# jamornsriwasansak/evplp

Hardware: AMD Instinct MI355X
Metric: Mpaths/s (higher is better)
Workload: dtype f32

## Files before the change

### evplp_amd/csrc/device_common.hpp

```cpp
#pragma once
#include "evplp_types.h"
#include "ev_math.h"

namespace evplp {

#define EV_PI 3.14159265358979323846f
#define EV_INV_PI 0.318309886183790671537767526745028724068919291480912897495f
#define EV_DEV __device__ __forceinline__

struct V3 { float x, y, z; };
EV_DEV V3 v3(float x, float y, float z) { V3 r; r.x = x; r.y = y; r.z = z; return r; }
EV_DEV V3 v3(const float *p) { return v3(p[0], p[1], p[2]); }
EV_DEV V3 v3(float4 a) { return v3(a.x, a.y, a.z); }
EV_DEV V3 operator+(V3 a, V3 b) { return v3(a.x + b.x, a.y + b.y, a.z + b.z); }
EV_DEV V3 operator-(V3 a, V3 b) { return v3(a.x - b.x, a.y - b.y, a.z - b.z); }
EV_DEV V3 operator-(V3 a) { return v3(-a.x, -a.y, -a.z); }
EV_DEV V3 operator*(V3 a, V3 b) { return v3(a.x * b.x, a.y * b.y, a.z * b.z); }
EV_DEV V3 operator*(V3 a, float s) { return v3(a.x * s, a.y * s, a.z * s); }
EV_DEV V3 operator/(V3 a, float s) { return v3(a.x / s, a.y / s, a.z / s); }
EV_DEV float dot(V3 a, V3 b) { return a.x * b.x + a.y * b.y + a.z * b.z; }
EV_DEV V3 cross(V3 a, V3 b) { return v3(a.y * b.z - a.z * b.y, a.z * b.x - a.x * b.z, a.x * b.y - a.y * b.x); }
EV_DEV V3 normalize(V3 v) { float inv = 1.0f / sqrtf(dot(v, v)); return v * inv; }
EV_DEV V3 reflect(V3 i, V3 n) { float d = dot(n, i); return i - (n * 2.0f) * d; }
EV_DEV V3 faceforward(V3 n, V3 i, V3 nref) { return n * copysignf(1.0f, dot(i, nref)); }
// ... 386 lines not shown
        "v_pk_fma_f32 " T0 ", %[hx], %[pb], " T0 " op_sel:[0,1,0] op_sel_hi:[1,1,1]\n\t"                                                                                     \
        "v_pk_fma_f32 " T1 ", %[hy], %[pc], " T1 " op_sel:[0,0,0] op_sel_hi:[1,0,1]\n\t"                                                                                     \
        "v_pk_fma_f32 " T2 ", %[hz], %[pc], " T2 " op_sel:[0,1,0] op_sel_hi:[1,1,1]\n\t"                                                                                     \
        "v_max3_f32 " T3L ", " T3L ", " T4L ", " T5L " clamp\n\t"                                                                            \
        "v_min3_f32 " T0L ", " T0L ", " T1L ", " T2L " clamp\n\t"                                                                            \
        "v_max3_f32 " T3H ", " T3H ", " T4H ", " T5H " clamp\n\t"                                                                            \
        "v_min3_f32 " T0H ", " T0H ", " T1H ", " T2H " clamp\n\t"                                                                            \
        "v_cmp_lt_f32 vcc, " T3L ", " T0L "\n\t"                                                                                             \
        "v_cmp_lt_f32 %[m1], " T3H ", " T0H "\n\t"                                                                                           \
        "s_or_b64 %[t64], vcc, %[m1]\n\t"                                                                                                    \
        "s_cbranch_scc0 L_pop%=\n\t"                                                                                                         \
        "s_cmp_eq_u64 vcc, 0\n\t"                                                                                                            \
        "s_cbranch_scc1 L_c1%=\n\t"                                                                                                          \
        "s_cmp_eq_u64 %[m1], 0\n\t"                                                                                                          \
        "s_cbranch_scc1 L_c0%=\n\t"                                                                                                          \
        "s_bcnt1_i32_b64 %[p0], vcc\n\t"                                                                                                     \
        "s_bcnt1_i32_b64 %[p1], %[m1]\n\t"                                                                                                   \
        "s_cmp_ge_i32 %[p0], %[p1]\n\t"                                                                                                      \
        "s_cselect_b32 %[p0], %[c1], %[c0]\n\t"                                                                                              \
        "s_cselect_b32 %[cur], %[c0], %[c1]\n\t"                                                                                             \
        "s_mov_b32 m0, %[sp]\n\t"                                                                                                            \
        "s_add_i32 %[sp], %[sp], 1\n\t"                                                                                                      \
        "v_writelane_b32 %[vstack], %[p0], m0\n\t"                                                                                           \
        "s_branch L_end%=\n"                                                                                                                 \
        "L_c0%=:\n\t"                                                                                                                        \
        "s_mov_b32 %[cur], %[c0]\n\t"                                                                                                        \
        "s_branch L_end%=\n"                                                                                                                 \
        "L_c1%=:\n\t"                                                                                                                        \
        "s_mov_b32 %[cur], %[c1]\n\t"                                                                                                        \
        "s_branch L_end%=\n"                                                                                                                 \
        "L_pop%=:\n\t"                                                                                                                       \
        "s_brev_b32 %[cur], 1\n\t"                                                                                                           \
        "s_cmp_eq_u32 %[sp], 0\n\t"                                                                                                          \
        "s_cbranch_scc1 L_end%=\n\t"                                                                                                         \
        "s_sub_i32 %[sp], %[sp], 1\n\t"                                                                                                      \
        "s_nop 0\n\t"                                                                                                                        \
        "v_readlane_b32 %[cur], %[vstack], %[sp]\n"                                                                                          \
        "L_end%=:\n"                                                                                                                         \
        : [cur] "+s"(cur), [sp] "+s"(sp), [vstack] "+v"(vstack), [m1] "=&s"(m1_), [t64] "=&s"(t64_), [p0] "=&s"(p0_), [p1] "=&s"(p1_)          \
        : [cx] NC(cx_), [cy] NC(cy_), [cz] NC(cz_), [hx] NC(hx_), [hy] NC(hy_), [hz] NC(hz_), [c0] "s"(c0_), [c1] "s"(c1_),              \
          [pa] "v"(pa_), [pb] "v"(pb_), [pc] "v"(pc_),                                     \
          [pd] "v"(pd_), [pe] "v"(pe_), [lane] "v"(lane_id)                                                                 \
        : "vcc", "scc", "m0", T0L, T0H, T1L, T1H, T2L, T2H, T3L, T3H, T4L, T4H, T5L, T5H)

template <int VT = 0, bool CUT = false>
EV_DEV bool occluded_wave(const char *node_base, const char *leaf_base, V3 o, V3 d, float tmin, float tmax, bool alive_lane, WalkStats *ws = nullptr, const char *cut = nullptr, uint32_t cut_off = 0u,
                          const float4 *cut_lds = nullptr) {
    unsigned long long alive = ballot64(alive_lane), hitm = 0ull;
    if (alive == 0ull) return false;
    uint32_t cut_end = 0u;
    constexpr bool kCutLds = CUT && VT != 0 && EVPLP_WALK_ASM && !EVPLP_TRAVERSAL_STATS;
    if constexpr (kCutLds) {
        const int32_t nsyn = __builtin_amdgcn_readfirstlane(__float_as_int(cut_lds[3].z));
        if (nsyn == 0) return false;
        cut_off = 0u; cut_end = (uint32_t)nsyn;
    } else if constexpr (CUT) {
        int32_t nsyn;
        asm volatile("s_load_dword %0, %1, %2 offset:0x38\n\ts_waitcnt lgkmcnt(0)" : "=s"(nsyn) : "s"(cut), "s"(cut_off) : "memory");
        if (nsyn == 0) return false;
        cut_end = cut_off + ((uint32_t)nsyn << 6);
    }
    const V3 inv0 = v3(safe_rcp(d.x), safe_rcp(d.y), safe_rcp(d.z));
    const float ku = 1.0f / (tmax - tmin);
    const V3 inv = inv0 * ku;
    const v2f ivx = bc(inv.x), ivy = bc(inv.y), ivz = bc(inv.z);
    const v2f avx = bc(fabsf(inv.x)), avy = bc(fabsf(inv.y)), avz = bc(fabsf(inv.z));
    const float dead = __builtin_inff();
    v2f nox = bc(alive_lane ? (-(o.x * inv0.x) - tmin) * ku : dead), noy = bc(alive_lane ? (-(o.y * inv0.y) - tmin) * ku : dead),
        noz = bc(alive_lane ? (-(o.z * inv0.z) - tmin) * ku : dead);
    int sp = 0;
    int vstack = 0;
    int32_t cur = 0;
#if EVPLP_WALK_ASM && !EVPLP_TRAVERSAL_STATS
    if constexpr (VT != 0) {
        static_assert(VT == 52 || VT == 116, "reserved temporaries: v[52:63] or v[116:127]");
        const int lane_id = (int)(threadIdx.x & 63u);
        v2f pa_, pb_, pc_, pd_, pe_;
        pa_.x = ivx.x; pa_.y = ivy.x; pb_.x = ivz.x; pb_.y = avx.x; pc_.x = avy.x; pc_.y = avz.x;
        pd_.x = nox.x; pd_.y = noy.x; pe_.x = noz.x; pe_.y = noz.x;
#define EV_VISIT(N)                                                                                                                          \
        {                                                                                                                                    \
            const v2f cx_ = pk(N[0], N[1]), cy_ = pk(N[2], N[3]), cz_ = pk(N[4], N[5]), hx_ = pk(N[6], N[7]), hy_ = pk(N[8], N[9]), hz_ = pk(N[10], N[11]); \
            const int32_t c0_ = N[12], c1_ = N[13];                                                                                          \
            unsigned long long m1_, t64_; int32_t p0_, p1_;                                                                                  \
            if constexpr (VT == 52) EV_WALK_VISIT_ASM("v[52:53]", "v[54:55]", "v[56:57]", "v[58:59]", "v[60:61]", "v[62:63]", "v52", "v53", "v54", "v55", "v56", "v57", "v58", "v59", "v60", "v61", "v62", "v63"); \
            else EV_WALK_VISIT_ASM("v[116:117]", "v[118:119]", "v[120:121]", "v[122:123]", "v[124:125]", "v[126:127]", "v116", "v117", "v118", "v119", "v120", "v121", "v122", "v123", "v124", "v125", "v126", "v127"); \
        }
        for (;;) {
            if constexpr (CUT) {
                if (cut_off >= cut_end) break;
                v16i syn;
                {
                    const float4 *q = cut_lds + 4u * cut_off;
#pragma unroll
                    for (int w = 0; w < 4; w++) {
                        const float4 qq = q[w];
                        if (w < 3 || true) { syn[4 * w] = __builtin_amdgcn_readfirstlane(__float_as_int(qq.x)); syn[4 * w + 1] = __builtin_amdgcn_readfirstlane(__float_as_int(qq.y)); }
                        if (w < 3) { syn[4 * w + 2] = __builtin_amdgcn_readfirstlane(__float_as_int(qq.z)); syn[4 * w + 3] = __builtin_amdgcn_readfirstlane(__float_as_int(qq.w)); }
                    }
                    syn[14] = 0; syn[15] = 0;
                }
                cut_off++;
                EV_VISIT(syn)
            }
            for (;;) {
                while (cur >= 0) {
                    const v16i n = sload16(node_base, (uint32_t)cur << 6);
                    EV_VISIT(n)
                }
                if (cur == kNoChild) break;
                const uint32_t cnt = (((uint32_t)~cur) & 3u) + 1u, loff = (((uint32_t)~cur) >> 2) * 192u;
                bool any;
// ... 448 lines not shown
```

### evplp_amd/csrc/kernels.h

```cpp
#pragma once
#include "evplp_types.h"

namespace evplp {

struct PrimaryArgs {
    SceneDev sc; StripDev st; CamBasis cam;
    float jitter[2]; int32_t clear_light; int32_t pad;
    float4 *g_pos, *g_nrm, *g_dif, *g_phg, *g_light;
    float4 *tile_box;
    const char *cuts; int32_t cut_gw_log2, cut_gh_log2, cut_groups_x, pad2;
};
struct PrimaryCutArgs {
    const BvhNode *nodes; StripDev st; CamBasis cam;
    int32_t tiles_x, tiles_y, gw_log2, gh_log2, groups_x, groups_y;
    char *cuts;
};
void launch_primary_cuts(const PrimaryCutArgs &a, hipStream_t s);

struct LightTraceArgs {
    SceneDev sc;
    uint32_t rng_seed, path_begin, path_count, photons_per_path;
    evplp_record *records;
    int32_t *stack_overflow;
    uint32_t overflow_stride, pad;
};
#ifndef EVPLP_LT_STACK
#define EVPLP_LT_STACK 20
#endif
constexpr int kLtLdsStack = EVPLP_LT_STACK;
inline int lt_overflow_entries(const SceneDev &sc) {
    const int generic = 3 * ((sc.bvh_depth + 1) / 2) + 4;
    const int worst = sc.stack4_entries > 0 && sc.stack4_entries < generic ? sc.stack4_entries : generic;
    return worst > kLtLdsStack ? worst - kLtLdsStack : 0;
}

struct PassCounters {
    unsigned long long rays;
    unsigned long long nodes;
    unsigned long long pairs;
    unsigned long long aux;
    unsigned long long hist[64];
    unsigned long long shard_rays[64], shard_shaded[64];
    unsigned long long nonfinite;
};
#ifndef EVPLP_DEBUG_NAN
#define EVPLP_DEBUG_NAN 0
#endif
constexpr int kCounterShards = 64;

struct GatherArgs {
    SceneDev sc; StripDev st;
    const float4 *g_pos, *g_nrm, *g_dif, *g_phg;
    const evplp_record *vpls;
    const uint32_t *vpl_src_index;
    const uint32_t *nvpl;
    evplp_frame_params fp;
    float pdf_mc2; int32_t pad0;
    float4 *out;
    float4 *partial;
    size_t partial_stride;
    PassCounters *counters;
    int32_t splits_per_wave;
    int32_t block_h_log2;
    int32_t group_first, group_count;
    unsigned long long *vsl_masks; int32_t masks_per_split; int32_t pad1;
    const char *cuts; uint32_t cut_vpl_stride; int32_t cut_gw_log2, cut_gh_log2, cut_groups_x;
    int32_t band_first, band_rows, cut_group_row_first;
    int32_t item_deal;
    unsigned long long *block_cost;
};
struct AdaptArgs { const int4 *tiles; const float4 *snap; int32_t n1, pad; };
constexpr int kCutEntries = 8;
constexpr int kCutNodes = kCutEntries / 2;
constexpr int kCutSlotBytes = kCutNodes * 64;
struct CutArgs {
    const BvhNode *nodes;
    const float4 *tile_box;
    int32_t tiles_x, tiles_y;
    int32_t gw_log2, gh_log2;
    int32_t groups_x, groups_y;
    int32_t group_row_first, pad;
    const evplp_record *vpls; const uint32_t *nvpl; uint32_t vpl_stride;
    char *cuts;
    const int4 *adapt_tiles;
};
void launch_gather_cuts(const CutArgs &a, hipStream_t s);
void launch_tile_boxes(const StripDev &st, const float4 *g_pos, float4 *tile_box, int tiles_x, int tiles_y, hipStream_t s);
#ifndef EVPLP_VPL_SPLIT
#define EVPLP_VPL_SPLIT 128
#endif
constexpr int kVplSplit = EVPLP_VPL_SPLIT;
#ifndef EVPLP_GATHER_K
#define EVPLP_GATHER_K 2
#endif
constexpr int kDefaultSplitsPerWave = EVPLP_GATHER_K;

struct PathTraceArgs {
    SceneDev sc; StripDev st;
    const float4 *g_pos, *g_nrm, *g_dif, *g_phg;
    float camera_pos[3]; uint32_t rng_seed;
    uint32_t max_bounces, do_accumulate;
    float4 *out;
    PassCounters *counters;
};

constexpr int kPtBatchMaxSamples = 64;
constexpr size_t kPtBatchSlotBytes = 4 * 64 * sizeof(float4);
struct PtBatchSamples { float jitter[kPtBatchMaxSamples][2]; uint32_t seed[kPtBatchMaxSamples]; };
struct PtBatchChunk {
    const int32_t *list, *count;
    int32_t tiles;
    int32_t entry_first, entry_count, sample_first, sample_count, pad;
    float4 *staging;
    unsigned long long cut_mask;
};
void launch_pt_batch_list(const int4 *tiles, int32_t ntiles, int32_t *list, int32_t *count, hipStream_t s);
void launch_pt_batch_primary(const PrimaryArgs &a, const PtBatchSamples &sm, const PtBatchChunk &ch, hipStream_t s);
void launch_pt_batch_trace(const PathTraceArgs &a, const PtBatchSamples &sm, const PtBatchChunk &ch, hipStream_t s);
void launch_pt_batch_reduce(const StripDev &st, float4 *out, const PtBatchChunk &ch, hipStream_t s);
void launch_pt_batch_rescale(const StripDev &st, float4 *out, const AdaptArgs &ad, int32_t ntiles, hipStream_t s);

constexpr int kPtBudgetMaxTiles = 1 << 25;
struct PtBudgetChunk {
    const uint32_t *table; const int32_t *total;
    int32_t item_first, item_count;
    float4 *staging;
    unsigned long long cut_mask;
// ... 115 lines not shown
```

### evplp_amd/csrc/kernels_cut.hip

```cpp
#include "device_common.hpp"
#include "kernels.h"

namespace evplp {

struct CutFrustum {
    V3 p;
    float lo[3], hi[3];
    V3 pl[4]; float tol[4];
    bool planes;
};
EV_DEV bool cut_outside(const CutFrustum &F, const float c[3], const float h[3]) {
    bool out = false;
#pragma unroll
    for (int k = 0; k < 3; k++) out = out || (c[k] - h[k] > F.hi[k]) || (c[k] + h[k] < F.lo[k]);
    if (F.planes) {
        const V3 rel = v3(c[0] - F.p.x, c[1] - F.p.y, c[2] - F.p.z);
        const float mag = fabsf(rel.x) + fabsf(rel.y) + fabsf(rel.z) + h[0] + h[1] + h[2];
#pragma unroll
        for (int q = 0; q < 4; q++) {
            const V3 n = F.pl[q];
            const float far = __builtin_fmaf(fabsf(n.z), h[2], __builtin_fmaf(fabsf(n.y), h[1], __builtin_fmaf(fabsf(n.x), h[0], __builtin_fmaf(n.z, rel.z, __builtin_fmaf(n.y, rel.y, n.x * rel.x)))));
            out = out || (__builtin_fmaf(mag, F.tol[q], far) < 0.0f);
        }
    }
// ... 76 lines not shown
#pragma unroll
                for (int e = 0; e < 2; e++) {
                    if (2 * s2 + e < count) box_of(order[2 * s2 + e], c[e], h[e], r[e]);
                    else { r[e] = kNoChild; c[e][0] = c[e][1] = c[e][2] = 0.f; h[e][0] = h[e][1] = h[e][2] = -3.0e38f; }
                }
                out[4 * s2 + 0] = make_float4(c[0][0], c[1][0], c[0][1], c[1][1]);
                out[4 * s2 + 1] = make_float4(c[0][2], c[1][2], h[0][0], h[1][0]);
                out[4 * s2 + 2] = make_float4(h[0][1], h[1][1], h[0][2], h[1][2]);
                out[4 * s2 + 3] = make_float4(__int_as_float(r[0]), __int_as_float(r[1]), __int_as_float(nsyn), 0.f);
            }
        }
    }
}

template <bool ADAPT = false>
__global__ __launch_bounds__(64) void gather_cut_kernel(CutArgs a) {
    __shared__ int32_t s_ref[kCutRing][64];
    __shared__ uint32_t s_src[kCutRing][64];
    const int lane = threadIdx.x;
    const uint32_t nvpl = *a.nvpl;
    const uint32_t i = blockIdx.x % a.vpl_stride, gb = blockIdx.x / a.vpl_stride;
    if (i >= nvpl) return;
    const int gblocks_x = (a.groups_x + 7) >> 3;
    const int gx = (int)(gb % (uint32_t)gblocks_x) * 8 + (lane & 7), gyl = (int)(gb / (uint32_t)gblocks_x) * 8 + (lane >> 3);
    bool live = gx < a.groups_x && gyl < a.groups_y;
    if constexpr (ADAPT) {
        if (live) {
            const int gw = 1 << a.gw_log2, gh = 1 << a.gh_log2, gyi = a.group_row_first + gyl;
            bool retired = true;
            for (int ty = gyi * gh; ty < min((gyi + 1) * gh, a.tiles_y); ty++)
                for (int tx = gx * gw; tx < min((gx + 1) * gw, a.tiles_x); tx++) retired = retired && a.adapt_tiles[ty * a.tiles_x + tx].x != 0;
            live = !retired;
        }
    }
    if (__builtin_amdgcn_ballot_w64(live) == 0ull) return;
    const uint32_t g = (uint32_t)(min(gyl, a.groups_y - 1) * a.groups_x + min(gx, a.groups_x - 1));
    const int gy = a.group_row_first + min(gyl, a.groups_y - 1);
    const int gxc = min(gx, a.groups_x - 1);
    const float4 pv = reinterpret_cast<const float4 *>(a.vpls + i)[0];
    CutFrustum F; F.p = v3(pv.x, pv.y, pv.z);

    const int gw = 1 << a.gw_log2, gh = 1 << a.gh_log2;
    float ulo[3] = { 3.0e38f, 3.0e38f, 3.0e38f }, uhi[3] = { -3.0e38f, -3.0e38f, -3.0e38f };
    for (int ty = gy * gh; ty < min((gy + 1) * gh, a.tiles_y); ty++)
        for (int tx = gxc * gw; tx < min((gxc + 1) * gw, a.tiles_x); tx++) {
            const float4 lo = a.tile_box[2 * (ty * a.tiles_x + tx)], hi = a.tile_box[2 * (ty * a.tiles_x + tx) + 1];
            if (lo.x > hi.x) continue;
            ulo[0] = fminf(ulo[0], lo.x); ulo[1] = fminf(ulo[1], lo.y); ulo[2] = fminf(ulo[2], lo.z);
            uhi[0] = fmaxf(uhi[0], hi.x); uhi[1] = fmaxf(uhi[1], hi.y); uhi[2] = fmaxf(uhi[2], hi.z);
        }
    const bool any_tile = ulo[0] <= uhi[0];
    char *const slot = a.cuts + ((size_t)g * a.vpl_stride + i) * (size_t)kCutSlotBytes;
    if (live && !any_tile) reinterpret_cast<float4 *>(slot)[3] = make_float4(0.f, 0.f, 0.f, 0.f);
    const bool work = live && any_tile;
    if (!any_tile) { ulo[0] = ulo[1] = ulo[2] = 0.f; uhi[0] = uhi[1] = uhi[2] = 0.f; }
    {
        const float pp[3] = { F.p.x, F.p.y, F.p.z };
#pragma unroll
        for (int k = 0; k < 3; k++) {
            const float t0 = 0.0001f, t1 = 1.0f - 0.0001f;
            const float a0 = pp[k] * (1.0f - t0) + t0 * ulo[k], b0 = pp[k] * (1.0f - t0) + t0 * uhi[k];
            const float a1 = pp[k] * (1.0f - t1) + t1 * ulo[k], b1 = pp[k] * (1.0f - t1) + t1 * uhi[k];
            const float l = fminf(a0, a1), h = fmaxf(b0, b1);
            const float pad = 1.0e-5f * ((h - l) + fabsf(l) + fabsf(h)) + 1.0e-30f;
            F.lo[k] = l - pad; F.hi[k] = h + pad;
        }
    }
    {
        const V3 cen = v3(0.5f * (ulo[0] + uhi[0]), 0.5f * (ulo[1] + uhi[1]), 0.5f * (ulo[2] + uhi[2]));
        V3 m = cen - F.p;
        const float ml2 = dot(m, m);
        bool planes = ml2 > 1.0e-30f;
        m = m * __builtin_amdgcn_rsqf(fmaxf(ml2, 1.0e-30f));
        const V3 ax = fabsf(m.x) < 0.6f ? v3(1.f, 0.f, 0.f) : v3(0.f, 1.f, 0.f);
        V3 u = cross(m, ax); u = u * __builtin_amdgcn_rsqf(fmaxf(dot(u, u), 1.0e-30f));
        const V3 w = cross(m, u);
        float amin = 3.0e38f, amax = -3.0e38f, bmin = 3.0e38f, bmax = -3.0e38f;
#pragma unroll
        for (int q = 0; q < 8; q++) {
            const V3 d = v3(((q & 1) ? uhi[0] : ulo[0]) - F.p.x, ((q & 2) ? uhi[1] : ulo[1]) - F.p.y, ((q & 4) ? uhi[2] : ulo[2]) - F.p.z);
            const float dw = dot(m, d), dl2 = dot(d, d);
            if (!(dw > 0.0f) || dw * dw <= 0.0025f * dl2) planes = false;
            const float r = __builtin_amdgcn_rcpf(dw);
            const float ca = dot(u, d) * r, cb = dot(w, d) * r;
            amin = fminf(amin, ca); amax = fmaxf(amax, ca); bmin = fminf(bmin, cb); bmax = fmaxf(bmax, cb);
        }
        const float oa = 1.0e-4f * (1.0f + fmaxf(fabsf(amin), fabsf(amax))), ob = 1.0e-4f * (1.0f + fmaxf(fabsf(bmin), fabsf(bmax)));
        amin -= oa; amax += oa; bmin -= ob; bmax += ob;
        F.planes = planes;
        F.pl[0] = u - m * amin; F.pl[1] = m * amax - u; F.pl[2] = w - m * bmin; F.pl[3] = m * bmax - w;
#pragma unroll
        for (int q = 0; q < 4; q++) F.tol[q] = 4.0e-6f * (fabsf(F.pl[q].x) + fabsf(F.pl[q].y) + fabsf(F.pl[q].z));
    }

    cut_descend_and_store(a.nodes, F, slot, work, lane, s_ref, s_src);
}

__global__ __launch_bounds__(64) void primary_cut_kernel(PrimaryCutArgs a) {
    __shared__ int32_t s_ref[kCutRing][64];
    __shared__ uint32_t s_src[kCutRing][64];
    const int lane = threadIdx.x;
    const int gblocks_x = (a.groups_x + 7) >> 3;
    const int gx = (int)(blockIdx.x % (uint32_t)gblocks_x) * 8 + (lane & 7), gy = (int)(blockIdx.x / (uint32_t)gblocks_x) * 8 + (lane >> 3);
    const bool live = gx < a.groups_x && gy < a.groups_y;
    const int gxc = min(gx, a.groups_x - 1), gyc = min(gy, a.groups_y - 1);
    const int gw = 8 << a.gw_log2, gh = 8 << a.gh_log2;
    const int x0 = gxc * gw, x1 = min(x0 + gw, a.st.W) - 1;
// ... 30 lines not shown
```

### evplp_amd/csrc/kernels_gather.hip

```cpp
#include "device_common.hpp"
#include "kernels.h"
#include <algorithm>

namespace evplp {

constexpr int kRecF4 = sizeof(evplp_record) / 16;

struct Pixel {
    V3 p1, n1, rd, rs; float e; V3 wi10;
};

struct Vpl {
    V3 pos, n, flux, fdir, rd, rs; float psel, e;
};
EV_DEV Vpl load_vpl(const float4 *r) {
    Vpl v; float4 a = r[0], b = r[1], c = r[2], d = r[3], e = r[4], f = r[5];
    v.pos = v3(a); v.n = v3(b); v.psel = b.w; v.flux = v3(c); v.fdir = v3(d); v.rd = v3(e); v.rs = v3(f); v.e = f.w;
    return v;
}

EV_DEV float phong_eval_f_hw(V3 out, V3 in, V3 n, float e) {
    V3 r = reflect(-in, n);
    float d = fmaxf(dot(out, r), 0.0f);
    if (d <= 0.000001f) return 0.0f;
// ... 88 lines not shown
    return t;
}

template <bool RANGE = false>
EV_DEV uint32_t item_texel(const GatherArgs &a, int lane, int b) {
    const StripDev &st = a.st;
    const ItemIx ix = item_index<RANGE>(a, b);
    const int x = ix.tx * 8 + (lane & 7), ly = ix.ty * 8 + (lane >> 3);
    return (uint32_t)max(min(ly, st.local_rows - 1), 0) * (uint32_t)st.W + (uint32_t)min(x, st.W - 1);
}

EV_DEV uint32_t item_cut_group(const GatherArgs &a, const Item &t) {
    const int tx = __builtin_amdgcn_readfirstlane(t.x) >> 3, ty = __builtin_amdgcn_readfirstlane(t.ly) >> 3;
    return (uint32_t)(((ty >> a.cut_gh_log2) - a.cut_group_row_first) * a.cut_groups_x + (tx >> a.cut_gw_log2));
}
EV_DEV bool tile_retired(const GatherArgs &a, const AdaptArgs &ad, const Item &t) {
    const int tx = __builtin_amdgcn_readfirstlane(t.x) >> 3, ty = __builtin_amdgcn_readfirstlane(t.ly) >> 3;
    const uint32_t off = (uint32_t)(ty * ((a.st.W + 7) >> 3) + tx) * (uint32_t)sizeof(int4);
    int nt;
    asm volatile("s_load_dword %0, %1, %2\n\ts_waitcnt lgkmcnt(0)" : "=s"(nt) : "s"(ad.tiles), "s"(off) : "memory");
    return nt != 0;
}

#ifndef EVPLP_CUT_RING
#define EVPLP_CUT_RING 3
#endif
#ifndef EVPLP_PX_LDS
#define EVPLP_PX_LDS 1
#endif
constexpr int kGatherPxFloats = 64 * (EVPLP_PX_LDS ? 10 : 3);
#ifndef EVPLP_GATHER_WAVES
#define EVPLP_GATHER_WAVES 8
#endif

EV_DEV Vpl fetch_vpl(const evplp_record *r) {
    const v16i ra = *reinterpret_cast<const v16i *>(r);
    const v8i rb = *reinterpret_cast<const v8i *>(reinterpret_cast<const int *>(r) + 16);
    Vpl v;
    v.pos = v3(f_of(ra[0]), f_of(ra[1]), f_of(ra[2])); v.n = v3(f_of(ra[4]), f_of(ra[5]), f_of(ra[6])); v.psel = f_of(ra[7]);
    v.flux = v3(f_of(ra[8]), f_of(ra[9]), f_of(ra[10])); v.fdir = v3(f_of(ra[12]), f_of(ra[13]), f_of(ra[14]));
    v.rd = v3(f_of(rb[0]), f_of(rb[1]), f_of(rb[2])); v.rs = v3(f_of(rb[4]), f_of(rb[5]), f_of(rb[6])); v.e = f_of(rb[7]);
    return v;
}
EV_DEV void fetch_vpl_head(const evplp_record *vpls, uint32_t i, V3 &pos, V3 &n, float &psel) {
    const v8i ra = sload8(vpls, i * (uint32_t)sizeof(evplp_record));
    pos = v3(f_of(ra[0]), f_of(ra[1]), f_of(ra[2])); n = v3(f_of(ra[4]), f_of(ra[5]), f_of(ra[6])); psel = f_of(ra[7]);
}
EV_DEV void fetch_vpl_tail(const evplp_record *vpls, uint32_t i, Vpl &v) {
    const v16i rb = sload16(vpls, i * (uint32_t)sizeof(evplp_record) + 32u);
    v.flux = v3(f_of(rb[0]), f_of(rb[1]), f_of(rb[2])); v.fdir = v3(f_of(rb[4]), f_of(rb[5]), f_of(rb[6]));
    v.rd = v3(f_of(rb[8]), f_of(rb[9]), f_of(rb[10])); v.rs = v3(f_of(rb[12]), f_of(rb[13]), f_of(rb[14])); v.e = f_of(rb[15]);
}

#if EVPLP_GATHER_TIMES
__device__ unsigned long long g_gather_times[2 * 131072];
extern "C" int evplp_debug_gather_times(unsigned long long *out, int n) { return (int)hipMemcpyFromSymbol(out, HIP_SYMBOL(g_gather_times), sizeof(unsigned long long) * (size_t)n); }
#endif
EV_DEV void item_cost_add(const GatherArgs &a, int ty, unsigned long long t0, int waves) {
    const unsigned long long dt = __builtin_amdgcn_s_memrealtime() - t0;
    if (threadIdx.x == 0) atomicAdd(&a.block_cost[(ty * 8) / a.st.strip_rows], dt * 8ull / (unsigned long long)waves);
}
template <bool CUT, bool COST = false, bool ADAPT = false>
#if EVPLP_WALK_ASM && !EVPLP_TRAVERSAL_STATS
__attribute__((amdgpu_num_vgpr(52)))
#endif
__global__ __launch_bounds__(64, EVPLP_GATHER_WAVES) void gather_vpl_kernel(GatherArgs a, AdaptArgs ad) {
    unsigned long long t_cost = 0ull;
    if constexpr (COST) t_cost = __builtin_amdgcn_s_memrealtime();
#if EVPLP_GATHER_TIMES
    const unsigned long long t_start = __builtin_amdgcn_s_memrealtime();
#endif
    extern __shared__ float s_dyn[];
    float *const s_wi10 = s_dyn, *const s_lvl = s_dyn + kGatherPxFloats;
    const int lane = threadIdx.x;
    const Item t = item_setup(a, lane, (int)blockIdx.x);
    if (!t.has_tile) return;
    if constexpr (ADAPT) { if (tile_retired(a, ad, t)) return; }
    const uint32_t p = t.p;

    Pixel px;
    float4 gp = a.g_pos[p], gn = a.g_nrm[p], gd = a.g_dif[p], gs = a.g_phg[p];
    px.p1 = v3(gp); px.n1 = v3(gn); px.rd = v3(gd); px.rs = v3(gs); px.e = gs.w;
#ifndef EVPLP_WI10_LDS
#define EVPLP_WI10_LDS 1
#endif
    {
        const V3 w = normalize(v3(a.fp.camera_pos) - px.p1);
        s_wi10[lane] = w.x; s_wi10[64 + lane] = w.y; s_wi10[128 + lane] = w.z;
        px.wi10 = EVPLP_WI10_LDS ? v3(0.f, 0.f, 0.f) : w;
    }
    bool px_glossy = true;
    if constexpr (EVPLP_PX_LDS != 0) {
        static_assert(EVPLP_WI10_LDS != 0, "EVPLP_PX_LDS continues the LDS column of the view direction");
        s_wi10[192 + lane] = px.rd.x; s_wi10[256 + lane] = px.rd.y; s_wi10[320 + lane] = px.rd.z;
        s_wi10[384 + lane] = px.rs.x; s_wi10[448 + lane] = px.rs.y; s_wi10[512 + lane] = px.rs.z; s_wi10[576 + lane] = px.e;
        px_glossy = ballot64(px.rs.x != 0.0f || px.rs.y != 0.0f || px.rs.z != 0.0f) != 0ull;
        px.rd = v3(0.f, 0.f, 0.f); px.rs = v3(0.f, 0.f, 0.f); px.e = 0.0f;
    }
    const bool valid = t.in_image && gp.w != 0.0f;

    const uint32_t nvpl = *a.nvpl;
    const int k = a.splits_per_wave;
    const char *node_base = pinned(reinterpret_cast<const char *>(a.sc.nodes)), *leaf_base = pinned(reinterpret_cast<const char *>(a.sc.leaves));
    const evplp_record *vpls = pinned(a.vpls);
    const char *cuts_g = nullptr;
    if constexpr (CUT) cuts_g = pinned(a.cuts + (size_t)item_cut_group(a, t) * a.cut_vpl_stride * (size_t)kCutSlotBytes);
    V3 total = v3(0.f, 0.f, 0.f);
    uint32_t rays = t.in_image ? 0x80000000u : 0u, shaded = 0;
#if EVPLP_TRAVERSAL_STATS
    int32_t cache_leaf = kNoChild; bool prev_all_occ = false;
#endif
    constexpr bool kRing = CUT && EVPLP_WALK_ASM && !EVPLP_TRAVERSAL_STATS;
    constexpr int kRingSlots = EVPLP_CUT_RING, kAhead = kRingSlots - 1;
    __shared__ float4 s_cut[kRing ? kRingSlots : 1][kCutSlotBytes / 16];
    int pj = 0; uint32_t pi = (uint32_t)(t.group * k), qslot = 0u;
    auto ring_skip_empty = [&]() { while (pj < k && pi >= nvpl) { pj++; pi = (uint32_t)(t.group * k + pj); } };
    auto ring_issue = [&](uint32_t slot) {
        if (lane < kCutSlotBytes / 16) lds_dma16(cuts_g + (size_t)pi * kCutSlotBytes + (size_t)lane * 16u, lds_offset(&s_cut[slot][0]));
        pi += (uint32_t)kVplSplit; ring_skip_empty();
    };
    if constexpr (kRing) {
        ring_skip_empty();
        for (int q = 0; q < kAhead; q++) if (pj < k) ring_issue((uint32_t)q);
    }
    for (int jj = 0; jj < k; jj++) {
        const uint32_t split = (uint32_t)(t.group * k + jj);
        V3 result = v3(0.f, 0.f, 0.f);
        for (uint32_t i = split; i < nvpl; i += kVplSplit) {
            const float4 *cut_lds = nullptr;
            if constexpr (kRing) {
                if (pj < k) { ring_issue((qslot + (uint32_t)kAhead) % (uint32_t)kRingSlots); wait_vmcnt<kAhead>(); }
                else wait_vmcnt0();
                cut_lds = &s_cut[qslot][0];
                qslot = (qslot + 1u) % (uint32_t)kRingSlots;
            }
            V3 vpos, vn; float vpsel; fetch_vpl_head(vpls, i, vpos, vn, vpsel);
            V3 v12 = vpos - px.p1;
            float c1 = fmaxf(dot_exact(px.n1, v12), 0.0f);
            float c2 = fmaxf(-dot_exact(vn, v12), 0.0f);
            float c1c2 = c1 * c2;
            bool active = valid && !(c1c2 <= 0.0f);
            if (ballot64(active) == 0ull) continue;
            rays += active ? 1u : 0u;
            bool occ;
            {
#if EVPLP_TRAVERSAL_STATS
                unsigned long long cache_kill = 0ull;
                const unsigned long long act_m = ballot64(active);
                if (cache_leaf != kNoChild) {
                    const LeafOps L = fetch_leaf(leaf_base, (uint32_t)cache_leaf);
                    const V3 dd = -v12;
                    bool any = tri_pair_any(L.A, vpos, dd, 0.0001f, 1.0f - 0.0001f);
                    if (L.cnt > 2u) any = any | tri_pair_any(L.B, vpos, dd, 0.0001f, 1.0f - 0.0001f);
                    cache_kill = ballot64(any) & act_m;
                }
                WalkStats ws = { 0u, 0u, 0u, 0u, kNoChild, 0u };
                occ = occluded_wave<0, CUT>(node_base, leaf_base, vpos, -v12, 0.0001f, 1.0f - 0.0001f, active, &ws, cuts_g, i * (uint32_t)kCutSlotBytes);
                const bool all_occ = ballot64(active && !occ) == 0ull;
                const unsigned long long occ_m = ballot64(active && occ);
                if (lane == 0) {
                    atomicAdd(&a.counters->hist[41], (unsigned long long)__builtin_popcountll(occ_m));
                    atomicAdd(&a.counters->nodes, (unsigned long long)ws.nodes);
                    atomicAdd(&a.counters->aux, (unsigned long long)ws.syn);
                    atomicAdd(&a.counters->hist[min(ws.leaves, 31u)], 1ull);
                    atomicAdd(&a.counters->hist[32], 1ull);
                    atomicAdd(&a.counters->hist[33], (unsigned long long)ws.pairs);
                    if (all_occ) { atomicAdd(&a.counters->hist[34], 1ull); atomicAdd(&a.counters->hist[36], (unsigned long long)ws.nodes); atomicAdd(&a.counters->hist[37], (unsigned long long)ws.leaves); }
                    if (ws.leaves == 0u) atomicAdd(&a.counters->hist[35], (unsigned long long)ws.nodes);
                    if (cache_leaf != kNoChild) {
                        atomicAdd(&a.counters->hist[42], 1ull);
                        atomicAdd(&a.counters->hist[40], (unsigned long long)__builtin_popcountll(cache_kill));
                        if (cache_kill == act_m) { atomicAdd(&a.counters->hist[38], 1ull); atomicAdd(&a.counters->hist[39], (unsigned long long)ws.nodes); }
                        if (prev_all_occ) { atomicAdd(&a.counters->hist[44], 1ull); if (cache_kill == act_m) atomicAdd(&a.counters->hist[43], 1ull); }
                    }
                    atomicAdd(&a.counters->hist[45 + min(ws.nodes / 16u, 18u)], 1ull);
                }
                if (ws.hit_leaf != kNoChild) cache_leaf = ws.hit_leaf;
                prev_all_occ = all_occ;
#else
                occ = occluded_wave<EVPLP_WALK_ASM ? 52 : 0, CUT>(node_base, leaf_base, vpos, -v12, 0.0001f, 1.0f - 0.0001f, active, nullptr, cuts_g, i * (uint32_t)kCutSlotBytes, cut_lds);
#endif
            }
            const bool lit = active && !occ;
            if (ballot64(lit) == 0ull) continue;
            Vpl v; fetch_vpl_head(vpls, i, v.pos, v.n, v.psel); fetch_vpl_tail(vpls, i, v);
            evplp_frame_params fps; float pdf_mc2;
            {
                const void *ka = (const void *)__builtin_amdgcn_kernarg_segment_ptr();
                typedef int v4i_ __attribute__((ext_vector_type(4)));
                v4i_ q; int q2;
                asm volatile("s_load_dwordx4 %0, %2, %3\n\ts_load_dword %1, %2, %4\n\ts_waitcnt lgkmcnt(0)" : "=&s"(q), "=&s"(q2)
                             : "s"(ka), "s"((uint32_t)(offsetof(GatherArgs, fp) + offsetof(evplp_frame_params, mis_mode))), "s"((uint32_t)offsetof(GatherArgs, pdf_mc2)) : "memory");
                fps.mis_mode = (uint32_t)q[0]; fps.pdf_mc = f_of(q[1]); fps.clamping_value = f_of(q[2]); pdf_mc2 = f_of(q2);
            }
            if (lit) { result = result + vpl_shade<EVPLP_PX_LDS != 0>(fps, pdf_mc2, px, v, v12, c1c2, EVPLP_WI10_LDS ? s_wi10 + lane : nullptr, px_glossy); shaded++; }
        }
        {
            int lev = 0;
            while ((jj >> lev) & 1) {
                float *q = s_lvl + lev * 192 + lane;
                result = v3(q[0], q[64], q[128]) + result;
                lev++;
            }
            float *q = s_lvl + lev * 192 + lane;
            q[0] = result.x; q[64] = result.y; q[128] = result.z;
        }
        total = result;
    }
#if EVPLP_DEBUG_NAN
    if ((rays >> 31) != 0u && !(isfinite(total.x) && isfinite(total.y) && isfinite(total.z))) atomicAdd(&a.counters->nonfinite, 1ull);
#endif
#if EVPLP_XCD_TIMES
    if (lane == 0) atomicMax(&a.counters->hist[16 + (blockIdx.x & 7u)], (unsigned long long)__builtin_amdgcn_s_memrealtime());
#endif
#if EVPLP_GATHER_TIMES
    if (lane == 0 && (blockIdx.x & 15u) == 0u && (blockIdx.x >> 4) < 131072u) { g_gather_times[2 * (blockIdx.x >> 4)] = t_start; g_gather_times[2 * (blockIdx.x >> 4) + 1] = __builtin_amdgcn_s_memrealtime(); }
#endif
    int lane_out = lane, blk_out = (int)blockIdx.x;
    asm volatile("" : "+v"(lane_out), "+s"(blk_out));
    const bool in_image = (rays >> 31) != 0u;
    rays &= 0xffffu;
    if (in_image) a.partial[(size_t)item_index(a, blk_out).sg * a.partial_stride + item_texel(a, lane_out, blk_out)] = make_float4(total.x, total.y, total.z, __uint_as_float(rays | (shaded << 16)));
    if constexpr (COST) item_cost_add(a, item_index(a, blk_out).ty, t_cost, EVPLP_GATHER_WAVES);
}

EV_DEV float4 reduce_out(V3 r, float inv, float acc, float4 old) {
    return make_float4(r.x / inv + acc * old.x, r.y / inv + acc * old.y, r.z / inv + acc * old.z, 0.0f + acc * old.w);
}
template <bool ADAPT = false>
__global__ __launch_bounds__(256) void gather_reduce_kernel(GatherArgs a, int stencil_test, AdaptArgs ad) {
    const size_t i = (size_t)blockIdx.x * 256 + threadIdx.x;
    const size_t n = (size_t)a.st.W * a.st.local_rows;
    unsigned long long rays = 0ull, shaded = 0ull;
    bool writes = i < n;
    int nt = 0;
    if (writes) {
        const int ly = (int)(i / a.st.W);
        if (a.st.global_row(ly) >= a.st.H) writes = false;
        else {
            if constexpr (ADAPT) nt = ad.tiles[(ly >> 3) * ((a.st.W + 7) >> 3) + ((int)(i - (size_t)ly * a.st.W) >> 3)].x;
            if (nt == 0 && stencil_test && a.g_pos[i].w == 0.0f) writes = false;
        }
    }
    if (ADAPT && writes && nt != 0) {
        const float4 R = ad.snap[i];
        const double f = __ddiv_rn((double)ad.n1, (double)nt);
        a.out[i] = make_float4(__double2float_rn(__dmul_rn((double)R.x, f)), __double2float_rn(__dmul_rn((double)R.y, f)),
                               __double2float_rn(__dmul_rn((double)R.z, f)), __double2float_rn(__dmul_rn((double)R.w, f)));
// ... 259 lines not shown
}
EV_DEV int launch_tile(const GatherArgs &a) { return item_index<true>(a, (int)blockIdx.x).tile_l; }

template <bool CUT, bool COST = false, bool ADAPT = false>
#if EVPLP_WALK_ASM && !EVPLP_TRAVERSAL_STATS
__attribute__((amdgpu_num_vgpr(52)))
#endif
__global__ __launch_bounds__(64, EVPLP_GATHER_WAVES) void gather_vsl_walk_kernel(GatherArgs a, AdaptArgs ad) {
    unsigned long long t_cost = 0ull;
    if constexpr (COST) t_cost = __builtin_amdgcn_s_memrealtime();
    __shared__ unsigned long long s_lit[kVslChunk];
    const int lane = threadIdx.x;
    const Item t = item_setup<true>(a, lane, (int)blockIdx.x);
    if (!t.has_tile) return;
    if constexpr (ADAPT) { if (tile_retired(a, ad, t)) return; }
    const bool valid = t.in_image;
    const uint32_t nvpl = *a.nvpl;
    const int k = a.splits_per_wave;
    const char *node_base = pinned(reinterpret_cast<const char *>(a.sc.nodes)), *leaf_base = pinned(reinterpret_cast<const char *>(a.sc.leaves));
    const evplp_record *vpls = pinned(a.vpls);
    V3 p1, n1;
    { const float4 gp = a.g_pos[t.p], gn = a.g_nrm[t.p]; p1 = v3(gp); n1 = v3(gn); }
    const int tile_l = launch_tile(a);
    unsigned long long *masks = a.vsl_masks + vsl_mask_base(a, tile_l, t.group);
    const char *cuts_g = nullptr;
    if constexpr (CUT) cuts_g = pinned(a.cuts + (size_t)item_cut_group(a, t) * a.cut_vpl_stride * (size_t)kCutSlotBytes);
    uint32_t rays = 0;
    constexpr bool kRing = CUT && EVPLP_WALK_ASM && !EVPLP_TRAVERSAL_STATS;
    constexpr int kRingSlots = EVPLP_CUT_RING, kAhead = kRingSlots - 1;
    __shared__ float4 s_cut[kRing ? kRingSlots : 1][kCutSlotBytes / 16];
    int pj = 0; uint32_t pi = (uint32_t)(t.group * k), qslot = 0u;
    auto ring_skip_empty = [&]() { while (pj < k && pi >= nvpl) { pj++; pi = (uint32_t)(t.group * k + pj); } };
    auto ring_issue = [&](uint32_t slot) {
        if (lane < kCutSlotBytes / 16) lds_dma16(cuts_g + (size_t)pi * kCutSlotBytes + (size_t)lane * 16u, lds_offset(&s_cut[slot][0]));
        pi += (uint32_t)kVplSplit; ring_skip_empty();
    };
    if constexpr (kRing) {
        ring_skip_empty();
        for (int q = 0; q < kAhead; q++) if (pj < k) ring_issue((uint32_t)q);
    }
    for (int jj = 0; jj < k; jj++) {
        const uint32_t split = (uint32_t)(t.group * k + jj);
        uint32_t cbase = 0;
        for (uint32_t first = split; first < nvpl; first += (uint32_t)(kVplSplit * kVslChunk), cbase += (uint32_t)kVslChunk) {
            const uint32_t n = min((uint32_t)kVslChunk, (nvpl - first + (uint32_t)kVplSplit - 1u) / (uint32_t)kVplSplit);
            for (uint32_t c = 0; c < n; c++) {
                const uint32_t i = first + c * (uint32_t)kVplSplit;
                const float4 *cut_lds = nullptr;
                if constexpr (kRing) {
                    if (pj < k) { ring_issue((qslot + (uint32_t)kAhead) % (uint32_t)kRingSlots); wait_vmcnt<kAhead>(); }
                    else wait_vmcnt0();
                    cut_lds = &s_cut[qslot][0];
                    qslot = (qslot + 1u) % (uint32_t)kRingSlots;
                }
                V3 vpos, vn; float vpsel; fetch_vpl_head(vpls, i, vpos, vn, vpsel);
                const V3 v12 = vpos - p1;
                const float d2 = dot(v12, v12), a1 = fmaxf(dot(n1, v12), 0.0f), a2 = fmaxf(-dot(vn, v12), 0.0f);
                const float quick = a1 * a2 * __builtin_amdgcn_rcpf(d2);
                bool pre = valid && (quick > 0.000000001f);
                if (ballot64(valid && fabsf(quick - 0.000000001f) <= 0.000000000001f) != 0ull) {
                    const float dist = sqrtf(d2);
                    const V3 nv12 = v12 / dist;
                    const float c1c2 = fmaxf(dot(n1, nv12), 0.0f) * fmaxf(-dot(vn, nv12), 0.0f);
                    pre = valid && !(c1c2 <= 0.000000001f);
                }
                unsigned long long lit = 0ull;
                if (ballot64(pre) != 0ull) {
                    rays += pre ? 1u : 0u;
                    const bool occ = occluded_wave<EVPLP_WALK_ASM ? 52 : 0, CUT>(node_base, leaf_base, vpos, -v12, 0.0001f, 1.0f - 0.0001f, pre, nullptr, cuts_g, i * (uint32_t)kCutSlotBytes, cut_lds);
                    lit = ballot64(pre && !occ);
                }
                if (lane == 0) s_lit[c] = lit;
            }
            unsigned long long *dst = masks + (size_t)jj * a.masks_per_split + cbase;
            for (uint32_t q = (uint32_t)lane; q < n; q += 64u) dst[q] = s_lit[q];
        }
    }
#if EVPLP_XCD_TIMES
    if (lane == 0) atomicMax(&a.counters->hist[24 + (blockIdx.x & 7u)], (unsigned long long)__builtin_amdgcn_s_memrealtime());
#endif
    for (int off = 32; off > 0; off >>= 1) rays += __shfl_down(rays, off);
    if (lane == 0 && rays != 0u) atomicAdd(&a.counters->shard_rays[blockIdx.x & (kCounterShards - 1)], (unsigned long long)rays);
    if constexpr (COST) item_cost_add(a, item_index<true>(a, (int)blockIdx.x).ty, t_cost, EVPLP_GATHER_WAVES);
}

template <bool COST = false, bool ADAPT = false>
__global__ __launch_bounds__(64, EVPLP_VSL_WAVES) void gather_vsl_shade_kernel(GatherArgs a, AdaptArgs ad) {
    unsigned long long t_cost = 0ull;
    if constexpr (COST) t_cost = __builtin_amdgcn_s_memrealtime();
    extern __shared__ float s_lvl[];
    __shared__ unsigned long long s_lit[kVslChunk];
    const int lane = threadIdx.x;
    const int W = a.st.W;
    const Item t = item_setup<true>(a, lane, (int)blockIdx.x);
    if (!t.has_tile) return;
    if constexpr (ADAPT) { if (tile_retired(a, ad, t)) return; }
    const bool valid = t.in_image;
    const uint32_t pixel_id = (uint32_t)t.gy * (uint32_t)W + (uint32_t)t.x;
    const uint64_t pixel_key = vsl_key(((uint64_t)a.fp.rng_seed << 32) | (uint64_t)pixel_id);
    const uint32_t nvpl = *a.nvpl;
    const int k = a.splits_per_wave;
    const evplp_record *vpls = pinned(a.vpls);
    const int tile_l = launch_tile(a);
    const unsigned long long *masks = a.vsl_masks + vsl_mask_base(a, tile_l, t.group);
    Pixel px;
    { const float4 gp = a.g_pos[t.p], gn = a.g_nrm[t.p], gd = a.g_dif[t.p], gs = a.g_phg[t.p]; px.p1 = v3(gp); px.n1 = v3(gn); px.rd = v3(gd); px.rs = v3(gs); px.e = gs.w; }
    px.wi10 = normalize(v3(a.fp.camera_pos) - px.p1);
    VslPixel P;
    {
        const float ml = max_color(px.rd), mp = max_color(px.rs);
        P.dead = ml + mp <= 0.000001f; P.psel = ml / (mp + ml);
        P.glossy = px.rs.x != 0.0f || px.rs.y != 0.0f || px.rs.z != 0.0f; P.pdf_glossy = !(px.rs.x <= 0.000001f);
        P.R1 = reflect(-px.wi10, px.n1);
    }
    V3 total = v3(0.f, 0.f, 0.f);
    uint32_t cnt = 0;
    for (int jj = 0; jj < k; jj++) {
        const uint32_t split = (uint32_t)(t.group * k + jj);
        V3 result = v3(0.f, 0.f, 0.f);
        uint32_t cbase = 0;
        for (uint32_t first = split; first < nvpl; first += (uint32_t)(kVplSplit * kVslChunk), cbase += (uint32_t)kVslChunk) {
            const uint32_t n = min((uint32_t)kVslChunk, (nvpl - first + (uint32_t)kVplSplit - 1u) / (uint32_t)kVplSplit);
            uint32_t moff = (uint32_t)jj * (uint32_t)a.masks_per_split + cbase;
            asm volatile("" : "+s"(moff));
            const unsigned long long *src = masks + moff;
            uint32_t q0 = (uint32_t)lane;
            asm volatile("" : "+v"(q0));
            for (uint32_t q = q0; q < n; q += 64u) s_lit[q] = src[q];
            for (uint32_t c = 0; c < n; c++) {
                const unsigned long long lit = s_lit[c];
                const uint32_t lo = __builtin_amdgcn_readfirstlane((uint32_t)lit), hi = __builtin_amdgcn_readfirstlane((uint32_t)(lit >> 32));
                if ((lo | hi) == 0u) continue;
                const uint32_t i = first + c * (uint32_t)kVplSplit;
                Vpl v; fetch_vpl_head(vpls, i, v.pos, v.n, v.psel); fetch_vpl_tail(vpls, i, v);
                const bool lit_lane = (((lane < 32 ? lo : hi) >> (lane & 31)) & 1u) != 0u;
                const uint64_t record_key = vsl_key((uint64_t)(1u + a.vpl_src_index[i]) * 0xD1B54A32D192ED03ull);
                const bool diffuse_wave = !(v.rs.x != 0.0f || v.rs.y != 0.0f || v.rs.z != 0.0f) && ballot64(lit_lane && (P.glossy || P.psel < 1.0f)) == 0ull;
                if (lit_lane) {
                    const V3 v12 = v.pos - px.p1;
                    const float inv_dist = vslm::rsq(dot(v12, v12));
                    const V3 nv12 = v12 * inv_dist;
                    VslCtx cx;
                    const float rdratio = a.fp.vsl_radius * inv_dist;
                    cx.half_cone = (rdratio >= 1.0f) ? EV_PI / 2.0f : asinf(rdratio);
                    cx.cos_half_cone = (rdratio >= 1.0f) ? cosf(EV_PI / 2.0f) : vslm::fsqrt(1.0f - rdratio * rdratio);
                    cx.solid_angle = EV_PI * 2.0f * (1.0f - cx.cos_half_cone);
                    cx.inv_solid_angle = vslm::rcp(cx.solid_angle);
                    cx.inv_pi_r2 = a.fp.vsl_inv_pi_radius2; cx.nd12 = nv12;
                    const int num_samples = (int)(cx.half_cone / EV_PI * 2.0f * 100.0f) + 1;
                    cnt += ((uint32_t)num_samples << 12) + 1u;
                    VslRng rng = vsl_rng_seed(pixel_key, record_key);
                    VslLight L;
                    {
                        const float ml = max_color(v.rd), mp = max_color(v.rs);
                        L.dead = ml + mp <= 0.000001f; L.psel = ml * vslm::rcp(mp + ml);
                        L.glossy = v.rs.x != 0.0f || v.rs.y != 0.0f || v.rs.z != 0.0f; L.pdf_glossy = !(v.rs.x <= 0.000001f);
                        L.R2 = reflect(-v.fdir, v.n);
                    }
                    VslFrames F;
                    F.nd_n1 = onb_local(vslm::fonb_make(px.n1), nv12); F.nd_r1 = onb_local(vslm::fonb_make(P.R1), nv12);
                    F.nd_n2 = onb_local(vslm::fonb_make(v.n), -nv12);  F.nd_r2 = onb_local(vslm::fonb_make(L.R2), -nv12);
                    const Onb cone = vslm::fonb_make(nv12);
                    V3 acc = v3(0.f, 0.f, 0.f);
                    if (diffuse_wave) {
                        float acc_d = 0.0f;
                        for (int sidx = 0; sidx < num_samples; sidx++) {
                            vsl_sample_cone<true>(px, v, P, L, cx, cone, acc, acc_d, rng);
                            vsl_sample_brdf1<true>(px, v, P, L, cx, F, acc, rng);
                            vsl_sample_brdf2<true>(px, v, P, L, cx, F, acc, rng);
                        }
                        acc = acc + ((px.rd * EV_INV_PI) * (v.rd * EV_INV_PI)) * acc_d;
                    } else {
                        float unused = 0.0f;
                        for (int sidx = 0; sidx < num_samples; sidx++) {
                            vsl_sample_cone<false>(px, v, P, L, cx, cone, acc, unused, rng);
                            vsl_sample_brdf1<false>(px, v, P, L, cx, F, acc, rng);
                            vsl_sample_brdf2<false>(px, v, P, L, cx, F, acc, rng);
                        }
                    }
                    acc = (v.flux * cx.inv_pi_r2) * acc;
                    result = result + acc * vslm::rcp((float)num_samples);
                }
            }
        }
        {
            int lev = 0;
            while ((jj >> lev) & 1) {
// ... 77 lines not shown
```

Before: 42660.

## Cull back-facing VPL/tile pairs in cut pass and batch VPL scalar loads

The cut-building kernel now tests whether a VPL's normal faces away from the whole tile box. If so, it writes a negative sentinel into the cut slot and the wave exits early when no lane has work. The gather kernels read that sentinel from LDS and skip the VPL entirely, avoiding the vertex math and occlusion walk. Separately, the shading fetch merges the VPL record load, kernarg loads and a prefetch of the next VPL head into one scalar-load batch, and the glossy flag is made wave-uniform. This adds a conservative-tolerance culling test and more scalar register pressure, at some risk to exactness near grazing normals.

Result: no change. 43030, median of 6 (+0.9%).

```diff
diff --git a/evplp_amd/csrc/device_common.hpp b/evplp_amd/csrc/device_common.hpp
--- a/evplp_amd/csrc/device_common.hpp
+++ b/evplp_amd/csrc/device_common.hpp
@@ -462,12 +462,12 @@
     constexpr bool kCutLds = CUT && VT != 0 && EVPLP_WALK_ASM && !EVPLP_TRAVERSAL_STATS;
     if constexpr (kCutLds) {
         const int32_t nsyn = __builtin_amdgcn_readfirstlane(__float_as_int(cut_lds[3].z));
-        if (nsyn == 0) return false;
+        if (nsyn <= 0) return false;
         cut_off = 0u; cut_end = (uint32_t)nsyn;
     } else if constexpr (CUT) {
         int32_t nsyn;
         asm volatile("s_load_dword %0, %1, %2 offset:0x38\n\ts_waitcnt lgkmcnt(0)" : "=s"(nsyn) : "s"(cut), "s"(cut_off) : "memory");
-        if (nsyn == 0) return false;
+        if (nsyn <= 0) return false;
         cut_end = cut_off + ((uint32_t)nsyn << 6);
     }
     const V3 inv0 = v3(safe_rcp(d.x), safe_rcp(d.y), safe_rcp(d.z));
diff --git a/evplp_amd/csrc/kernels.h b/evplp_amd/csrc/kernels.h
--- a/evplp_amd/csrc/kernels.h
+++ b/evplp_amd/csrc/kernels.h
@@ -73,6 +73,10 @@
 constexpr int kCutEntries = 8;
 constexpr int kCutNodes = kCutEntries / 2;
 constexpr int kCutSlotBytes = kCutNodes * 64;
+constexpr int32_t kCutDead = -1;
+#ifndef EVPLP_DEAD_PAIRS
+#define EVPLP_DEAD_PAIRS 1
+#endif
 struct CutArgs {
     const BvhNode *nodes;
     const float4 *tile_box;
diff --git a/evplp_amd/csrc/kernels_cut.hip b/evplp_amd/csrc/kernels_cut.hip
--- a/evplp_amd/csrc/kernels_cut.hip
+++ b/evplp_amd/csrc/kernels_cut.hip
@@ -152,7 +152,23 @@
     const bool any_tile = ulo[0] <= uhi[0];
     char *const slot = a.cuts + ((size_t)g * a.vpl_stride + i) * (size_t)kCutSlotBytes;
     if (live && !any_tile) reinterpret_cast<float4 *>(slot)[3] = make_float4(0.f, 0.f, 0.f, 0.f);
-    const bool work = live && any_tile;
+    bool dead = false;
+    if (EVPLP_DEAD_PAIRS != 0 && any_tile) {
+        const float4 nv = reinterpret_cast<const float4 *>(a.vpls + i)[1];
+        const float nn[3] = { nv.x, nv.y, nv.z }, pp[3] = { F.p.x, F.p.y, F.p.z };
+        float msum = 0.0f, n1 = 0.0f, mag = 0.0f;
+        bool all_nonpos = true;
+#pragma unroll
+        for (int k = 0; k < 3; k++) {
+            const float mk = fmaxf(nn[k] * (ulo[k] - pp[k]), nn[k] * (uhi[k] - pp[k]));
+            all_nonpos = all_nonpos && mk <= 0.0f;
+            msum += mk; n1 += fabsf(nn[k]); mag += fabsf(pp[k]) + fmaxf(fabsf(ulo[k]), fabsf(uhi[k]));
+        }
+        dead = all_nonpos || msum < -(1.0e-6f * n1 * mag + 1.0e-30f);
+    }
+    if (live && dead) reinterpret_cast<float4 *>(slot)[3] = make_float4(0.f, 0.f, __int_as_float(kCutDead), 0.f);
+    const bool work = live && any_tile && !dead;
+    if (__builtin_amdgcn_ballot_w64(work) == 0ull) return;
     if (!any_tile) { ulo[0] = ulo[1] = ulo[2] = 0.f; uhi[0] = uhi[1] = uhi[2] = 0.f; }
     {
         const float pp[3] = { F.p.x, F.p.y, F.p.z };
diff --git a/evplp_amd/csrc/kernels_gather.hip b/evplp_amd/csrc/kernels_gather.hip
--- a/evplp_amd/csrc/kernels_gather.hip
+++ b/evplp_amd/csrc/kernels_gather.hip
@@ -164,6 +164,43 @@
     v.rd = v3(f_of(rb[8]), f_of(rb[9]), f_of(rb[10])); v.rs = v3(f_of(rb[12]), f_of(rb[13]), f_of(rb[14])); v.e = f_of(rb[15]);
 }
 
+EV_DEV void fetch_vpl_record(const evplp_record *vpls, uint32_t i, Vpl &v) {
+    v8i ra; v16i rb;
+    asm("s_load_dwordx8 %0, %2, %3\n\ts_load_dwordx16 %1, %2, %3 offset:0x20\n\ts_waitcnt lgkmcnt(0)" : "=&s"(ra), "=&s"(rb) : "s"(vpls), "s"(i * (uint32_t)sizeof(evplp_record)));
+    v.pos = v3(f_of(ra[0]), f_of(ra[1]), f_of(ra[2])); v.n = v3(f_of(ra[4]), f_of(ra[5]), f_of(ra[6])); v.psel = f_of(ra[7]);
+    v.flux = v3(f_of(rb[0]), f_of(rb[1]), f_of(rb[2])); v.fdir = v3(f_of(rb[4]), f_of(rb[5]), f_of(rb[6]));
+    v.rd = v3(f_of(rb[8]), f_of(rb[9]), f_of(rb[10])); v.rs = v3(f_of(rb[12]), f_of(rb[13]), f_of(rb[14])); v.e = f_of(rb[15]);
+}
+#ifndef EVPLP_SHADE_BATCH
+#define EVPLP_SHADE_BATCH 1
+#endif
+#ifndef EVPLP_HEAD_AHEAD
+#define EVPLP_HEAD_AHEAD 1
+#endif
+static_assert(EVPLP_SHADE_BATCH != 0 || EVPLP_HEAD_AHEAD == 0, "the next head rides in the shading batch");
+constexpr uint32_t kNoVpl = 0xffffffffu;
+typedef int v4i __attribute__((ext_vector_type(4)));
+template <bool AHEAD>
+EV_DEV void fetch_vpl_shading(const evplp_record *vpls, uint32_t i, uint32_t next, Vpl &v, evplp_frame_params &fps, float &pdf_mc2, v8i &next_head) {
+    const void *ka = (const void *)__builtin_amdgcn_kernarg_segment_ptr();
+    const uint32_t off = i * (uint32_t)sizeof(evplp_record), o_fp = (uint32_t)(offsetof(GatherArgs, fp) + offsetof(evplp_frame_params, mis_mode)), o_p2 = (uint32_t)offsetof(GatherArgs, pdf_mc2);
+    v4i rn, q; v16i rb; int q2;
+#if EVPLP_SHADE_BATCH
+    if constexpr (AHEAD) asm volatile("s_load_dwordx4 %0, %5, %6 offset:0x10\n\ts_load_dwordx16 %1, %5, %6 offset:0x20\n\ts_load_dwordx4 %2, %7, %8\n\ts_load_dword %3, %7, %9\n\t"
+                 "s_load_dwordx8 %4, %5, %10\n\ts_waitcnt lgkmcnt(0)" : "=&s"(rn), "=&s"(rb), "=&s"(q), "=&s"(q2), "=&s"(next_head)
+                 : "s"(vpls), "s"(off), "s"(ka), "s"(o_fp), "s"(o_p2), "s"((next != kNoVpl ? next : i) * (uint32_t)sizeof(evplp_record)) : "memory");
+    else asm volatile("s_load_dwordx4 %0, %4, %5 offset:0x10\n\ts_load_dwordx16 %1, %4, %5 offset:0x20\n\ts_load_dwordx4 %2, %6, %7\n\ts_load_dword %3, %6, %8\n\t"
+                 "s_waitcnt lgkmcnt(0)" : "=&s"(rn), "=&s"(rb), "=&s"(q), "=&s"(q2) : "s"(vpls), "s"(off), "s"(ka), "s"(o_fp), "s"(o_p2) : "memory");
+    v.n = v3(f_of(rn[0]), f_of(rn[1]), f_of(rn[2])); v.psel = f_of(rn[3]);
+    v.flux = v3(f_of(rb[0]), f_of(rb[1]), f_of(rb[2])); v.fdir = v3(f_of(rb[4]), f_of(rb[5]), f_of(rb[6]));
+    v.rd = v3(f_of(rb[8]), f_of(rb[9]), f_of(rb[10])); v.rs = v3(f_of(rb[12]), f_of(rb[13]), f_of(rb[14])); v.e = f_of(rb[15]);
+#else
+    fetch_vpl_head(vpls, i, v.pos, v.n, v.psel); fetch_vpl_tail(vpls, i, v);
+    asm volatile("s_load_dwordx4 %0, %2, %3\n\ts_load_dword %1, %2, %4\n\ts_waitcnt lgkmcnt(0)" : "=&s"(q), "=&s"(q2) : "s"(ka), "s"(o_fp), "s"(o_p2) : "memory");
+#endif
+    fps.mis_mode = (uint32_t)q[0]; fps.pdf_mc = f_of(q[1]); fps.clamping_value = f_of(q[2]); pdf_mc2 = f_of(q2);
+}
+
 #if EVPLP_GATHER_TIMES
 __device__ unsigned long long g_gather_times[2 * 131072];
 extern "C" int evplp_debug_gather_times(unsigned long long *out, int n) { return (int)hipMemcpyFromSymbol(out, HIP_SYMBOL(g_gather_times), sizeof(unsigned long long) * (size_t)n); }
@@ -218,7 +255,7 @@
     const char *cuts_g = nullptr;
     if constexpr (CUT) cuts_g = pinned(a.cuts + (size_t)item_cut_group(a, t) * a.cut_vpl_stride * (size_t)kCutSlotBytes);
     V3 total = v3(0.f, 0.f, 0.f);
-    uint32_t rays = t.in_image ? 0x80000000u : 0u, shaded = 0;
+    uint32_t rays = t.in_image ? 0x80000000u : 0u, shaded = CUT && px_glossy ? 0x80000000u : 0u;
 #if EVPLP_TRAVERSAL_STATS
     int32_t cache_leaf = kNoChild; bool prev_all_occ = false;
 #endif
@@ -235,6 +272,8 @@
         ring_skip_empty();
         for (int q = 0; q < kAhead; q++) if (pj < k) ring_issue((uint32_t)q);
     }
+    constexpr bool kHeadAhead = EVPLP_HEAD_AHEAD != 0 && CUT;
+    v8i head; uint32_t head_of = kNoVpl;
     for (int jj = 0; jj < k; jj++) {
         const uint32_t split = (uint32_t)(t.group * k + jj);
         V3 result = v3(0.f, 0.f, 0.f);
@@ -245,8 +284,12 @@
                 else wait_vmcnt0();
                 cut_lds = &s_cut[qslot][0];
                 qslot = (qslot + 1u) % (uint32_t)kRingSlots;
+                if (EVPLP_DEAD_PAIRS != 0 && __builtin_amdgcn_readfirstlane(__float_as_int(cut_lds[3].z)) < 0) continue;
             }
-            V3 vpos, vn; float vpsel; fetch_vpl_head(vpls, i, vpos, vn, vpsel);
+            if (head_of != i) head = sload8(vpls, i * (uint32_t)sizeof(evplp_record));
+            head_of = kNoVpl;
+            const V3 vpos = v3(f_of(head[0]), f_of(head[1]), f_of(head[2])), vn = v3(f_of(head[4]), f_of(head[5]), f_of(head[6]));
+            head = __builtin_nondeterministic_value(head);
             V3 v12 = vpos - px.p1;
             float c1 = fmaxf(dot_exact(px.n1, v12), 0.0f);
             float c2 = fmaxf(-dot_exact(vn, v12), 0.0f);
@@ -295,17 +338,14 @@
             }
             const bool lit = active && !occ;
             if (ballot64(lit) == 0ull) continue;
-            Vpl v; fetch_vpl_head(vpls, i, v.pos, v.n, v.psel); fetch_vpl_tail(vpls, i, v);
+            uint32_t next = i + (uint32_t)kVplSplit;
+            if (next >= nvpl) next = jj + 1 < k && split + 1u < nvpl ? split + 1u : kNoVpl;
+            Vpl v; v.pos = vpos;
             evplp_frame_params fps; float pdf_mc2;
-            {
-                const void *ka = (const void *)__builtin_amdgcn_kernarg_segment_ptr();
-                typedef int v4i_ __attribute__((ext_vector_type(4)));
-                v4i_ q; int q2;
-                asm volatile("s_load_dwordx4 %0, %2, %3\n\ts_load_dword %1, %2, %4\n\ts_waitcnt lgkmcnt(0)" : "=&s"(q), "=&s"(q2)
-                             : "s"(ka), "s"((uint32_t)(offsetof(GatherArgs, fp) + offsetof(evplp_frame_params, mis_mode))), "s"((uint32_t)offsetof(GatherArgs, pdf_mc2)) : "memory");
-                fps.mis_mode = (uint32_t)q[0]; fps.pdf_mc = f_of(q[1]); fps.clamping_value = f_of(q[2]); pdf_mc2 = f_of(q2);
-            }
-            if (lit) { result = result + vpl_shade<EVPLP_PX_LDS != 0>(fps, pdf_mc2, px, v, v12, c1c2, EVPLP_WI10_LDS ? s_wi10 + lane : nullptr, px_glossy); shaded++; }
+            fetch_vpl_shading<kHeadAhead>(vpls, i, next, v, fps, pdf_mc2, head);
+            if (kHeadAhead) head_of = next;
+            const bool glossy = CUT ? (__builtin_amdgcn_readfirstlane(shaded) >> 31) != 0u : px_glossy;
+            if (lit) { result = result + vpl_shade<EVPLP_PX_LDS != 0>(fps, pdf_mc2, px, v, v12, c1c2, EVPLP_WI10_LDS ? s_wi10 + lane : nullptr, glossy); shaded++; }
         }
         {
             int lev = 0;
@@ -671,6 +711,10 @@
                     else wait_vmcnt0();
                     cut_lds = &s_cut[qslot][0];
                     qslot = (qslot + 1u) % (uint32_t)kRingSlots;
+                    if (EVPLP_DEAD_PAIRS != 0 && __builtin_amdgcn_readfirstlane(__float_as_int(cut_lds[3].z)) < 0) {
+                        if (lane == 0) s_lit[c] = 0ull;
+                        continue;
+                    }
                 }
                 V3 vpos, vn; float vpsel; fetch_vpl_head(vpls, i, vpos, vn, vpsel);
                 const V3 v12 = vpos - p1;
@@ -751,7 +795,7 @@
                 const uint32_t lo = __builtin_amdgcn_readfirstlane((uint32_t)lit), hi = __builtin_amdgcn_readfirstlane((uint32_t)(lit >> 32));
                 if ((lo | hi) == 0u) continue;
                 const uint32_t i = first + c * (uint32_t)kVplSplit;
-                Vpl v; fetch_vpl_head(vpls, i, v.pos, v.n, v.psel); fetch_vpl_tail(vpls, i, v);
+                Vpl v; fetch_vpl_record(vpls, i, v);
                 const bool lit_lane = (((lane < 32 ? lo : hi) >> (lane & 31)) & 1u) != 0u;
                 const uint64_t record_key = vsl_key((uint64_t)(1u + a.vpl_src_index[i]) * 0xD1B54A32D192ED03ull);
                 const bool diffuse_wave = !(v.rs.x != 0.0f || v.rs.y != 0.0f || v.rs.z != 0.0f) && ballot64(lit_lane && (P.glossy || P.psel < 1.0f)) == 0ull;
```
